# Masthetheus/kmer-ml

Measured on NVIDIA B200. Metric: kmer_count_feature_throughput, higher is better.
Workload: dtype u32

## Files before the change

### kmerml_b200/csrc/api.cu

```cuda
#include <dlfcn.h>

#include <algorithm>
#include <atomic>
#include <condition_variable>
#include <cstdio>
#include <cstdlib>
#include <cstring>
#include <memory>
#include <mutex>
#include <new>
#include <string>
#include <thread>
#include <vector>

#include "internal.h"

namespace km {

static thread_local std::string g_err;
void set_error(const std::string& msg) { g_err = msg; }
int cuda_fail(cudaError_t e, const char* what) {
    g_err = std::string("CUDA error: ") + cudaGetErrorString(e) + " in " + what;
    return KMERML_ERR_CUDA;
}
// ... 229 lines not shown
    lm.scratch_stride = scratch_stride;
    if (scratch_stride) {
        rc = ws.scratch.ensure((size_t)scratch_stride * lm.scratch_slots * 4);
        if (rc) return rc;
    }
    lm.scratch = (uint32_t*)ws.scratch.p;

    const uint64_t total_bytes = h_offsets[n_genomes] - h_offsets[0];
    const uint64_t target = (uint64_t)ctx->sm_count * 8;
    uint64_t walked_bytes = total_bytes;
    if (range_end) walked_bytes = std::min(total_bytes, range_end > range_begin ? range_end - range_begin : 0);
    int part_tiles_per_slice = 1;
    {
        const uint64_t tiles = std::max<uint64_t>(walked_bytes / TILE_BYTES, 1);
        const uint64_t slots = (uint64_t)ctx->sm_count * 2;
        for (uint64_t w = 1;; w++) {
            const uint64_t t = (tiles * 100 + slots * w * 96 - 1) / (slots * w * 96);
            if (t <= (uint64_t)PART_MAX_TILES_PER_RUN) {
                part_tiles_per_slice = (int)std::max<uint64_t>(t, 1);
                break;
            }
        }
    }
    if (const char* e = getenv("KMERML_TILES_PER_RUN")) {
        const int v = atoi(e);
        if (v >= 1 && v <= PART_MAX_TILES_PER_RUN) part_tiles_per_slice = v;
    }
    std::vector<uint64_t> slice_bytes(n_genomes);
    std::vector<uint32_t> first_slice(n_genomes + 1);
    uint64_t n_slices = 0;
    for (int g = 0; g < n_genomes; g++) {
        uint64_t bytes = h_offsets[g + 1] - h_offsets[g];
        uint64_t sb;
        if (use_part) {
            sb = (uint64_t)TILE_BYTES * part_tiles_per_slice;
// ... 93 lines not shown
    const size_t row_bytes = (size_t)row.off[nk] * 4;
    if (use_part) {
        const int k_stop = std::max(kcount - PART_LOW_BASES, kmin);
        uint64_t max_group_runs = 0, max_group_bytes = 0, max_group_genomes = 0;
        for (size_t gi = 0, g0 = 0; gi < group_end.size(); g0 = group_end[gi], gi++) {
            max_group_runs = std::max<uint64_t>(max_group_runs, first_slice[group_end[gi]] - first_slice[g0]);
            max_group_bytes = std::max<uint64_t>(max_group_bytes, h_offsets[group_end[gi]] - h_offsets[g0]);
            max_group_genomes = std::max<uint64_t>(max_group_genomes, group_end[gi] - g0);
        }
        const int nb = 1 << (2 * (kcount - PART_LOW_BASES));
        const size_t payload_bytes = align_up((size_t)max_group_runs * run_payload_bytes, 256);
        const size_t nsec_bytes = align_up((size_t)max_group_runs * nb * 2, 256);
        const size_t ov_bytes = align_up((size_t)max_group_bytes * 4 + 64, 256);
        const size_t ovc_bytes = align_up((size_t)n_genomes * 8 + 8, 256);
        const size_t tl_bytes = align_up((size_t)((max_group_bytes >> 6) + 1024 * (max_group_genomes + 1)) * 8, 256);
        rc = ws.part.ensure(payload_bytes + nsec_bytes + ov_bytes + tl_bytes + ovc_bytes);
        if (rc) return rc;
        uint8_t* pw = (uint8_t*)ws.part.p;
        void* d_payload = pw;
        uint16_t* d_nsec = (uint16_t*)(pw + payload_bytes);
        uint32_t* d_overflow = (uint32_t*)(pw + payload_bytes + nsec_bytes);
        unsigned long long* d_tail_list = (unsigned long long*)(pw + payload_bytes + nsec_bytes + ov_bytes);
        unsigned int* d_ov_counts = (unsigned int*)(pw + payload_bytes + nsec_bytes + ov_bytes + tl_bytes);
        unsigned int* d_tail_counts = d_ov_counts + n_genomes;
        unsigned int* d_tail_any = d_tail_counts + n_genomes;
        KM_CUDA(cudaMemsetAsync(d_ov_counts, 0, (size_t)n_genomes * 8 + 8, s));
        for (int i = 0; i < nk; i++)
            if (row.k[i] < k_stop)
                KM_CUDA(cudaMemset2DAsync(d_counts + row.off[i], (size_t)counts_stride * 4, 0,
                                          (size_t)(1ull << (2 * row.k[i])) * 4, (size_t)n_genomes, s));
        if (scratch_stride && k_stop > kmin)
            KM_CUDA(cudaMemsetAsync(lm.scratch, 0, (size_t)scratch_stride * n_genomes * 4, s));
        int g0 = 0;
        for (size_t gi = 0; gi < group_end.size(); gi++) {
            const int g1 = group_end[gi], ng = g1 - g0;
            const int nt = (int)(first_slice[g1] - first_slice[g0]);
            const uint64_t batch_lo = h_offsets[g0];
            {
                Prof pr(ctx, s, 4, nt > 0 ? 1 : 0);
                rc = launch_partition(d_fasta, d_genomes, d_slices + first_slice[g0], nt, part_tiles_per_slice, kcount,
                                      kmin, min_rec, lm, d_stats, d_payload, d_nsec, d_overflow, d_ov_counts, batch_lo,
                                      d_tail_list, d_tail_counts, d_tail_any, (uint32_t)g0, s);
            }
            if (rc) return rc;
            {
                Prof pr(ctx, s, 5, 1);
                rc = launch_bucket(lm, row, kcount, kmin, d_gruns, part_tiles_per_slice, d_payload, d_nsec, d_stats,
                                   canonical ? nullptr : d_freq, freq_stride, d_totals, (uint32_t)g0, ng, s);
            }
            if (rc) return rc;
            if (kcount > kmin) {
                Prof pr(ctx, s, 3, canonical || !d_freq ? 2 : 4);
                rc = launch_tails(d_fasta, lm, row, kcount, kmin, min_rec, d_genomes, d_slices + first_slice[g0], nt,
                                  d_tail_list, d_tail_counts, d_tail_any, batch_lo, d_stats, canonical ? nullptr : d_freq, freq_stride,
                                  (uint32_t)g0, ng, s);
                if (rc) return rc;
            }
            for (int h0 = g0; h0 < g1; h0 += 32768) {
                const int nh = std::min(32768, g1 - h0);
                {
                    Prof pr(ctx, s, 3, canonical || !d_freq ? 1 : 2);
                    rc = launch_overflow(lm, row, kcount, kmin, d_genomes, d_overflow, d_ov_counts, batch_lo, d_stats,
                                         canonical ? nullptr : d_freq, freq_stride, (uint32_t)h0, nh, s);
// ... 1292 lines not shown
```

### kmerml_b200/csrc/dense.cu

```cuda
#include <algorithm>

#include "fasta_walk.cuh"
#include "internal.h"

namespace km {

struct DevTails {
    const LevelMap* lm;
    GenomeStats* st;
    uint32_t genome;
    __device__ __noinline__ void tail(int j, uint32_t idx) const {
        atomicAdd(lm->ptr(genome, j) + idx, 1u);
        atomicAdd(&st->n_tail[j], 1ull);
    }
};

struct NoTails {
    __device__ __forceinline__ void tail(int, uint32_t) const {}
};

struct TailList {
    unsigned long long* list;
    unsigned int* counts;
    unsigned int* any_full;
    uint64_t batch_lo;
    uint32_t genome0;
};
__device__ __forceinline__ unsigned long long* tail_list_of(const TailList& tl, const GenomeDev& gd, uint32_t g,
                                                            uint32_t* cap) {
    *cap = (uint32_t)((gd.hi - gd.file_lo) >> 6) + 1024u;
    return tl.list + ((gd.file_lo - tl.batch_lo) >> 6) + 1024ull * (g - tl.genome0);
}
struct ListTails {
    const LevelMap* lm;
    GenomeStats* st;
    uint32_t genome;
    int k_stop;
    unsigned long long* list;
    unsigned int* count;
    unsigned int* any_full;
    uint32_t cap;
    __device__ __noinline__ void tail(int j, uint32_t idx) const {
        atomicAdd(&st->n_tail[j], 1ull);
        if (j < k_stop) {
            atomicAdd(lm->ptr(genome, j) + idx, 1u);
            return;
        }
// ... 555 lines not shown
struct PartWalkSmem {
    uint32_t last16[COUNT_THREADS];
    uint8_t flags[2 * COUNT_THREADS];
    uint8_t clean[COUNT_THREADS];
};

template <int NB_SHIFT>
struct PartSmem {
    uint16_t staged[PartGeom<NB_SHIFT>::stage_entries];
    uint32_t cnt[PART_MAX_BUCKETS];
    uint16_t written[PART_MAX_BUCKETS];
    PartWalkSmem walk;
    unsigned long long carry[2];
    uint32_t prev_tile[2];
    unsigned long long sh_total;
};
static_assert(sizeof(PartSmem<10>) <= 113 * 1024, "two partition CTAs must fit in one SM's shared memory");

struct GenomeRuns {
    uint32_t run0, n_runs;
};

__device__ __forceinline__ void store_sector(uint4* dst, const uint4& a, const uint4& b) {
    asm volatile("st.global.v8.b32 [%0], {%1, %2, %3, %4, %5, %6, %7, %8};" ::"l"(dst), "r"(a.x), "r"(a.y), "r"(a.z),
                 "r"(a.w), "r"(b.x), "r"(b.y), "r"(b.z), "r"(b.w) : "memory");
}

template <int NB_SHIFT>
__device__ __noinline__ void flush_slot_slow(PartSmem<NB_SHIFT>& sm, uint32_t b, uint4* region, uint32_t cap,
                                             uint32_t* ov, unsigned int* ov_count) {
// ... 9 lines not shown
            region[((size_t)b * cap + wr) * 2 + 1] = slot[2 * q + 1];
            wr++;
        } else {
            overflow_push_sector(ov, ov_count, b, slot16 + q * PART_SECTOR);
        }
    }
    if (nfull && left) {
        const uint4 a = slot[2 * nfull], d = slot[2 * nfull + 1];
        slot[0] = a;
        slot[1] = d;
    }
    sm.written[b] = (uint16_t)wr;
    sm.cnt[b] = left;
}

template <int NB_SHIFT>
__global__ void __launch_bounds__(COUNT_THREADS, 2)
partition_kernel(const uint8_t* __restrict__ buf, const GenomeDev* __restrict__ gds,
                 const Slice* __restrict__ runs, DenseParams P, LevelMap lm,
                 GenomeStats* stats, uint4* __restrict__ payload, uint16_t* __restrict__ nsec, uint32_t cap,
                 uint32_t* __restrict__ overflow, unsigned int* __restrict__ ov_counts, uint64_t batch_lo,
                 TailList tl, int k_stop) {
    using G = PartGeom<NB_SHIFT>;
    constexpr uint32_t slot_size = G::slot_size;
    constexpr uint32_t nb = G::nb;
    constexpr uint32_t VPB = slot_size / 8;
    extern __shared__ __align__(16) unsigned char part_smem_raw[];
    PartSmem<NB_SHIFT>& sm = *reinterpret_cast<PartSmem<NB_SHIFT>*>(part_smem_raw);
    const int tid = threadIdx.x;
    const Slice sl = runs[blockIdx.x];
    const GenomeDev gd = gds[sl.genome];
    Genome g;
    g.b = buf;
    g.lo = gd.lo;
    g.hi = gd.hi;
    TileCtx tc;
    tc.flags = sm.walk.flags; tc.clean = sm.walk.clean; tc.last16 = sm.walk.last16;
    tc.carry = sm.carry; tc.prev_tile = sm.prev_tile;
    for (uint32_t i = tid; i < nb; i += COUNT_THREADS) { sm.cnt[i] = 0; sm.written[i] = 0; }
    if (tid == 0) sm.sh_total = 0;

    SlotSink<NB_SHIFT> sink;
    sink.cnt_s = (uint32_t)__cvta_generic_to_shared(sm.cnt);
    sink.staged_s = (uint32_t)__cvta_generic_to_shared(sm.staged);
    sink.ov = overflow + (gd.file_lo - batch_lo);
    sink.ov_count = ov_counts + sl.genome;
    sink.kmask = P.mask;
    sink.n = 0;
    ListTails tails;
    tails.lm = &lm; tails.st = stats + sl.genome; tails.genome = sl.genome; tails.k_stop = k_stop;
    tails.list = tail_list_of(tl, gd, sl.genome, &tails.cap);
    tails.count = tl.counts + sl.genome;
    tails.any_full = tl.any_full;
    uint4* const region = payload + (size_t)blockIdx.x * nb * cap * 2;
    walk_slice<false>(buf, g, sl, P, sink, tails, tc, [&](uint32_t) {
        uint4* st = reinterpret_cast<uint4*>(sm.staged);
        if (G::owned) {
#pragma unroll
            for (int h = 0; h < 2; h++) {
                const uint32_t b = (uint32_t)tid + h * COUNT_THREADS;
                const uint32_t c = sm.cnt[b];
                if (c < PART_SECTOR) continue;
                const uint32_t wr = sm.written[b];
                if (c > slot_size || wr + 3u > cap) {
                    flush_slot_slow<NB_SHIFT>(sm, b, region, cap, sink.ov, sink.ov_count);
                    continue;
                }
                const uint32_t sw = ((uint32_t)tid >> 2) & 1u, sx = sw ^ 1u;
                uint4* slot = st + b * VPB;
                uint4* dst = region + (b * cap + wr) * 2u;
                {
                    const uint4 x0 = slot[sw], x1 = slot[sx];
                    dst[sw] = x0;
                    dst[sx] = x1;
                }
                uint32_t mv = 2;
                if (c >= 2 * PART_SECTOR) {
                    const uint4 x0 = slot[2 + sw], x1 = slot[2 + sx];
                    dst[2 + sw] = x0;
                    dst[2 + sx] = x1;
                    mv = 4;
                    if (c == 3 * PART_SECTOR) {
                        const uint4 y0 = slot[4 + sw], y1 = slot[4 + sx];
                        dst[4 + sw] = y0;
                        dst[4 + sx] = y1;
                        mv = 0;
                    }
                }
                const uint4 m0 = slot[mv + sw], m1 = slot[mv + sx];
                slot[sw] = m0;
                slot[sx] = m1;
                sm.written[b] = (uint16_t)(wr + c / PART_SECTOR);
                sm.cnt[b] = c % PART_SECTOR;
            }
        } else {
#pragma unroll
            for (int j = 0; j < (int)(G::stage_entries / 8 / COUNT_THREADS); j++) {
                const uint32_t v = (uint32_t)tid + j * COUNT_THREADS;
                const uint32_t b = v / VPB, jv = v % VPB, q = jv >> 1;
                const uint32_t c = min(sm.cnt[b], slot_size);
                const uint32_t nfull = c / PART_SECTOR;
                const uint32_t wr = sm.written[b];
                const uint4 x = st[v];
                if (VPB <= 32) __syncwarp(); else __syncthreads();
                if (q < nfull) {
                    const uint32_t sec = wr + q;
                    if (sec < cap) region[(b * cap + sec) * 2u + (jv & 1u)] = x;
                    else if (!(jv & 1u)) overflow_push_sector(sink.ov, sink.ov_count, b, sm.staged + b * slot_size + q * PART_SECTOR);
                }
                if (VPB <= 32) __syncwarp(); else __syncthreads();
                if (q == nfull && nfull && (c % PART_SECTOR)) st[b * VPB + (jv & 1u)] = x;
                if (jv == 0) {
                    sm.cnt[b] = c % PART_SECTOR;
                    sm.written[b] = (uint16_t)min(wr + nfull, cap);
                }
            }
        }
    });
    __syncthreads();
    for (uint32_t b = tid; b < nb; b += COUNT_THREADS) {
        const uint32_t left = sm.cnt[b];
        uint32_t wr = sm.written[b];
        if (left) {
            uint32_t e[PART_SECTOR / 2];
            const uint16_t* src16 = sm.staged + (size_t)b * slot_size;
            const uint32_t* src = reinterpret_cast<const uint32_t*>(src16);
            if (wr < cap) {
#pragma unroll
                for (int i = 0; i < PART_SECTOR / 2; i++) {
                    uint32_t w = src[i];
                    const uint32_t pad = payload_pad(b, b * 16u + 2u * i);
                    if (2u * i >= left) w = (w & 0xFFFF0000u) | pad;
                    if (2u * i + 1u >= left) w = (w & 0x0000FFFFu) | ((pad ^ 1u) << 16);
                    e[i] = w;
                }
                uint4* dst = region + (b * cap + wr) * 2u;
                dst[0] = make_uint4(e[0], e[1], e[2], e[3]);
                dst[1] = make_uint4(e[4], e[5], e[6], e[7]);
                wr++;
            } else {
                for (uint32_t i = 0; i < left; i++)
                    overflow_push(sink.ov, sink.ov_count, (b << (2 * PART_LOW)) | (src16[i] & (uint32_t)(PART_BINS - 1)));
            }
        }
        nsec[(size_t)blockIdx.x * nb + b] = (uint16_t)wr;
    }
    const unsigned long long total = block_sum_u32(sink.n, &sm.sh_total);
    if (tid == 0 && total) atomicAdd(&stats[sl.genome].total_top, total);
}

struct LevelInfo {
    int ki[16];
};

constexpr int BUCKET_THREADS = 512;

constexpr int BUCKET_NS_CHUNK = 1024;
#ifndef KM_BUCKET_BULK_STORE
#define KM_BUCKET_BULK_STORE 1
#endif
struct BucketSmem {
    uint32_t hist[PART_BINS + 256];
    uint16_t ns[BUCKET_NS_CHUNK];
    unsigned long long tot[16];
    uint32_t* lvl_counts[16];
    float* lvl_freq[16];
    double lvl_inv[16];
};
constexpr int BUCKET_CTAS_PER_SM = 3;
static_assert(sizeof(BucketSmem) <= 75 * 1024, "three bucket CTAs must fit in one SM's shared memory");

__device__ __forceinline__ void bulk_store(void* dst, uint32_t src_smem, uint32_t bytes) {
    asm volatile("cp.async.bulk.global.shared::cta.bulk_group [%0], [%1], %2;" ::"l"(dst), "r"(src_smem), "r"(bytes) : "memory");
    asm volatile("cp.async.bulk.commit_group;" ::: "memory");
}
__device__ __forceinline__ void bulk_store_wait_read() { asm volatile("cp.async.bulk.wait_group.read 0;" ::: "memory"); }

__device__ __forceinline__ void hist_add8(uint32_t hbase, const uint4& x, uint32_t fix) {
    const uint32_t w[4] = {x.x ^ fix, x.y ^ fix, x.z ^ fix, x.w ^ fix};
#pragma unroll
    for (int i = 0; i < 4; i++) {
        asm volatile("red.shared.add.u32 [%0], 1;" ::"r"(hbase + ((w[i] & 0xFFFFu) << 2)) : "memory");
        asm volatile("red.shared.add.u32 [%0], 1;" ::"r"(hbase + ((w[i] >> 16) << 2)) : "memory");
    }
}

__global__ void __launch_bounds__(BUCKET_THREADS, BUCKET_CTAS_PER_SM)
bucket_kernel(LevelMap lm, RowSpec row, LevelInfo li, int k, int k_stop, const GenomeRuns* __restrict__ grs,
              const uint4* __restrict__ payload, const uint16_t* __restrict__ nsec, uint32_t cap,
              const GenomeStats* __restrict__ stats, float* freq, uint64_t freq_stride, uint64_t* totals,
              uint32_t genome0) {
    extern __shared__ __align__(16) unsigned char bucket_smem_raw[];
    BucketSmem& sm = *reinterpret_cast<BucketSmem*>(bucket_smem_raw);
    const int tid = threadIdx.x;
    const uint32_t b = blockIdx.x;
    const uint32_t nb = gridDim.x;
    const uint32_t g = genome0 + blockIdx.y;
    const GenomeRuns gr = grs[g];
    if (tid < row.nk) {
        const int j = row.k[tid];
        unsigned long long t = stats[g].total_top;
        for (int i = j; i < k; i++) t += stats[g].n_tail[i];
        sm.tot[tid] = t;
        if (totals && b == 0) totals[(uint64_t)g * row.nk + tid] = t;
    }
    __syncthreads();
    if (tid >= 32 && tid < 48) {
        const int level = tid - 32;
        uint32_t* cp = nullptr;
        float* fp = nullptr;
        double inv = 0.0;
        if (level >= k_stop && level <= k) {
// ... 12 lines not shown
    constexpr int PER1 = PART_BINS / 4 / BUCKET_THREADS;
    constexpr int PER2 = PART_BINS / 16 / BUCKET_THREADS;
    const uint32_t hbase = (uint32_t)__cvta_generic_to_shared(sm.hist);
    const uint32_t fix = payload_fix(b);
    {
        uint4* h4 = reinterpret_cast<uint4*>(sm.hist);
        for (int i = tid; i < (PART_BINS + 256) / 4; i += BUCKET_THREADS) h4[i] = make_uint4(0, 0, 0, 0);
    }
    constexpr int NWARP = BUCKET_THREADS / 32;
    const int lane = tid & 31, wid = tid >> 5;
    const size_t run_stride = (size_t)nb * cap * 2;
    for (uint32_t rb = 0; rb < gr.n_runs; rb += BUCKET_NS_CHUNK) {
        const uint32_t nr = min(gr.n_runs - rb, (uint32_t)BUCKET_NS_CHUNK);
        __syncthreads();
        for (uint32_t i = tid; i < nr; i += BUCKET_THREADS)
            sm.ns[i] = __ldg(nsec + (size_t)(gr.run0 + rb + i) * nb + b);
        __syncthreads();
        const uint4* base = payload + ((size_t)(gr.run0 + rb) * nb + b) * cap * 2;
        uint32_t r = wid, c = 0, nv = 0;
        auto settle = [&]() {
            while (r < nr && 32u * c >= (nv = 2u * sm.ns[r])) { r += NWARP; c = 0; }
        };
        auto issue = [&](uint4& x, bool& live) -> bool {
            settle();
            if (r >= nr) { live = false; return false; }
            const uint32_t v = 32u * c + lane;
            live = v < nv;
            if (live) x = __ldg(base + (size_t)r * run_stride + v);
            c++;
            return true;
        };
        uint4 x0, x1, x2, x3;
        bool l0, l1, l2, l3;
// ... 80 lines not shown
        float* fl = sm.lvl_freq[level];
        const double invl = sm.lvl_inv[level];
        for (int i = tid; i < n_next; i += 32) {
            const uint4 c = reinterpret_cast<const uint4*>(cur)[i];
            const uint32_t v = c.x + c.y + c.z + c.w;
            cl[i] = v;
            if (fl) fl[i] = (float)((double)v * invl);
            nxt[i] = v;
        }
        __syncwarp();
        uint32_t* t = cur; cur = nxt; nxt = t;
        n_cur = n_next;
    }
}

constexpr int OV_TABLE = 4096;
constexpr uint32_t OV_EMPTY = 0xFFFFFFFFu;

__global__ void __launch_bounds__(256)
overflow_kernel(LevelMap lm, RowSpec row, LevelInfo li, int k, int k_stop, const GenomeDev* __restrict__ gds,
                const uint32_t* __restrict__ overflow, const unsigned int* __restrict__ ov_counts, uint64_t batch_lo,
                const GenomeStats* __restrict__ stats, float* freq, uint64_t freq_stride, uint32_t genome0, int pass) {
    __shared__ uint32_t t_key[OV_TABLE];
    __shared__ uint32_t t_cnt[OV_TABLE];
    __shared__ unsigned int t_used;
    const uint32_t g = genome0 + blockIdx.y;
    const unsigned int n = ov_counts[g];
    if (blockIdx.x * 256u >= n) return;
    const uint32_t* ov = overflow + (gds[g].file_lo - batch_lo);
    const int tid = threadIdx.x;
// ... 315 lines not shown
                const uint32_t own = tile[t][A][B];
                out[b] = x < rc ? own + tile[p][Br][Ar] : (x == rc ? own : 0u);
            }
            *reinterpret_cast<uint4*>(c + x0) = make_uint4(out[0], out[1], out[2], out[3]);
            if (f)
                *reinterpret_cast<float4*>(f + x0) = make_float4((float)((double)out[0] * inv), (float)((double)out[1] * inv),
                                                                 (float)((double)out[2] * inv), (float)((double)out[3] * inv));
        }
    }
}

int dense_setup_attributes() {
    KM_CUDA(cudaFuncSetAttribute(count_kernel<1>, cudaFuncAttributeMaxDynamicSharedMemorySize,
                                 (1 << (2 * SMEM_MAX_K)) * 4));
    KM_CUDA(cudaFuncSetAttribute(count8_kernel, cudaFuncAttributeMaxDynamicSharedMemorySize, 32768 * 4));
    KM_CUDA(cudaFuncSetAttribute(partition_kernel<10>, cudaFuncAttributeMaxDynamicSharedMemorySize, (int)sizeof(PartSmem<10>)));
    KM_CUDA(cudaFuncSetAttribute(partition_kernel<8>, cudaFuncAttributeMaxDynamicSharedMemorySize, (int)sizeof(PartSmem<8>)));
    KM_CUDA(cudaFuncSetAttribute(partition_kernel<6>, cudaFuncAttributeMaxDynamicSharedMemorySize, (int)sizeof(PartSmem<6>)));
    KM_CUDA(cudaFuncSetAttribute(partition_kernel<4>, cudaFuncAttributeMaxDynamicSharedMemorySize, (int)sizeof(PartSmem<4>)));
    KM_CUDA(cudaFuncSetAttribute(bucket_kernel, cudaFuncAttributeMaxDynamicSharedMemorySize, (int)sizeof(BucketSmem)));
    return KMERML_OK;
}

int launch_prologue(const uint8_t* d_fasta, const uint64_t* d_offsets, GenomeDev* d_genomes,
                    GenomeStats* d_stats, int n_genomes, cudaStream_t s) {
    if (n_genomes <= 0) return KMERML_OK;
    prologue_kernel<<<(n_genomes + 127) / 128, 128, 0, s>>>(d_fasta, d_offsets, d_genomes, d_stats, n_genomes);
    KM_CUDA(cudaGetLastError());
    return KMERML_OK;
}

static DenseParams make_params(int k, int min_rec, bool tails, int tail_lo) {
    DenseParams P;
    P.k = k;
    P.mask = k >= 16 ? 0xFFFFFFFFu : ((1u << (2 * k)) - 1u);
// ... 27 lines not shown
        count_kernel<0><<<n_slices, COUNT_THREADS, 0, s>>>(d_fasta, d_genomes, d_slices, P, lm, d_stats, nullptr);
    }
    KM_CUDA(cudaGetLastError());
    return KMERML_OK;
}

uint32_t part_region_cap(int k, int tiles_per_run) {
    const uint32_t nb = 1u << (2 * (k - PART_LOW));
    return (uint32_t)tiles_per_run * (2u * TILE_BYTES / PART_SECTOR) / nb;
}

int launch_partition(const uint8_t* d_fasta, const GenomeDev* d_genomes, const Slice* d_runs, int n_runs,
                     int tiles_per_run, int k, int k_bottom, int min_rec, const LevelMap& lm,
                     GenomeStats* d_stats, void* d_payload, uint16_t* d_nsec, uint32_t* d_overflow,
                     unsigned int* d_ov_counts, uint64_t batch_lo, unsigned long long* d_tail_list,
                     unsigned int* d_tail_counts, unsigned int* d_tail_any, uint32_t genome0, cudaStream_t s) {
    if (n_runs <= 0) return KMERML_OK;
    DenseParams P = make_params(k, min_rec, k > k_bottom, k_bottom);
    const int k_stop = std::max(k - PART_LOW, k_bottom);
    const uint32_t cap = part_region_cap(k, tiles_per_run);
    TailList tl;
    tl.list = d_tail_list; tl.counts = d_tail_counts; tl.batch_lo = batch_lo; tl.genome0 = genome0;
    tl.any_full = d_tail_any;
#define KM_LAUNCH_PART(NBS)                                                                           \
    partition_kernel<NBS><<<n_runs, COUNT_THREADS, sizeof(PartSmem<NBS>), s>>>(                       \
        d_fasta, d_genomes, d_runs, P, lm, d_stats, (uint4*)d_payload, d_nsec, cap, d_overflow,       \
        d_ov_counts, batch_lo, tl, k_stop)
    switch (2 * (k - PART_LOW)) {
        case 10: KM_LAUNCH_PART(10); break;
        case 8: KM_LAUNCH_PART(8); break;
        case 6: KM_LAUNCH_PART(6); break;
        default: KM_LAUNCH_PART(4); break;
    }
#undef KM_LAUNCH_PART
    KM_CUDA(cudaGetLastError());
    return KMERML_OK;
}

static LevelInfo make_level_info(const RowSpec& row) {
    LevelInfo li;
    for (int j = 0; j < 16; j++) {
        li.ki[j] = -1;
        for (int i = 0; i < row.nk; i++)
            if (row.k[i] == j) li.ki[j] = i;
    }
    return li;
}

int launch_bucket(const LevelMap& lm, const RowSpec& row, int k, int k_bottom, const void* d_genome_runs,
                  int tiles_per_run, const void* d_payload, const uint16_t* d_nsec, const GenomeStats* d_stats,
                  float* d_freq, uint64_t freq_stride, uint64_t* d_totals, uint32_t genome0, int n_genomes,
                  cudaStream_t s) {
    if (n_genomes <= 0) return KMERML_OK;
    const int nb = 1 << (2 * (k - PART_LOW));
    const LevelInfo li = make_level_info(row);
    const int k_stop = std::max(k - PART_LOW, k_bottom);
    const uint32_t cap = part_region_cap(k, tiles_per_run);
    for (int h0 = 0; h0 < n_genomes; h0 += 32768) {
        dim3 grid((unsigned)nb, (unsigned)std::min(32768, n_genomes - h0));
        bucket_kernel<<<grid, BUCKET_THREADS, sizeof(BucketSmem), s>>>(lm, row, li, k, k_stop,
            (const GenomeRuns*)d_genome_runs, (const uint4*)d_payload, d_nsec, cap, d_stats, d_freq, freq_stride,
            d_totals, genome0 + (uint32_t)h0);
        KM_CUDA(cudaGetLastError());
    }
    return KMERML_OK;
}

int launch_overflow(const LevelMap& lm, const RowSpec& row, int k, int k_bottom, const GenomeDev* d_genomes,
                    const uint32_t* d_overflow, const unsigned int* d_ov_counts, uint64_t batch_lo,
                    const GenomeStats* d_stats, float* d_freq, uint64_t freq_stride, uint32_t genome0, int n_genomes,
                    cudaStream_t s) {
    if (n_genomes <= 0) return KMERML_OK;
    const LevelInfo li = make_level_info(row);
    const int k_stop = std::max(k - PART_LOW, k_bottom);
    dim3 grid(64, (unsigned)n_genomes);
    for (int pass = 0; pass < (d_freq ? 2 : 1); pass++) {
        overflow_kernel<<<grid, 256, 0, s>>>(lm, row, li, k, k_stop, d_genomes, d_overflow, d_ov_counts, batch_lo,
// ... 114 lines not shown
```

### kmerml_b200/csrc/internal.h

```cpp
#pragma once
#include <cuda_runtime.h>
#include <stdint.h>

#include <algorithm>
#include <functional>
#include <string>

#include "../../include/kmerml_b200.h"

namespace km {

void set_error(const std::string& msg);
int cuda_fail(cudaError_t e, const char* what);
#define KM_CUDA(expr)                                        \
    do {                                                     \
        cudaError_t e__ = (expr);                            \
        if (e__ != cudaSuccess) return ::km::cuda_fail(e__, #expr); \
    } while (0)

struct GenomeDev {
    uint64_t file_lo;
    uint64_t lo;
    uint64_t hi;
};
// ... 45 lines not shown
int launch_slice_headers(const uint8_t* d_fasta, const GenomeDev* d_genomes, Slice* d_slices, int n_slices,
                         cudaStream_t s);
int launch_count(const uint8_t* d_fasta, const GenomeDev* d_genomes, const Slice* d_slices,
                 int n_slices, int k, int k_bottom, int min_rec, bool use_smem, const LevelMap& lm,
                 GenomeStats* d_stats, cudaStream_t s);
int launch_cascade(const LevelMap& lm, int k_top, int k_bottom, uint32_t genome0, int n_genomes,
                   cudaStream_t s);
int cascade_launches(int k_top, int k_bottom);
int finalize_launches(const RowSpec& row, bool canonical);
int launch_finalize(const LevelMap& lm, const RowSpec& row, int k_top, bool canonical,
                    const GenomeStats* d_stats, float* d_freq, uint64_t freq_stride,
                    uint64_t* d_totals, uint32_t genome0, int n_genomes, cudaStream_t s);
constexpr int PART_MIN_K = 9, PART_MAX_K = 12, PART_LOW_BASES = 7;
constexpr int PART_STAGE_ENTRIES = 32768;
constexpr int PART_MAX_TILES_PER_RUN = 64;
uint32_t part_region_cap(int k, int tiles_per_run);
int launch_partition(const uint8_t* d_fasta, const GenomeDev* d_genomes, const Slice* d_runs, int n_runs,
                     int tiles_per_run, int k, int k_bottom, int min_rec, const LevelMap& lm,
                     GenomeStats* d_stats, void* d_payload, uint16_t* d_nsec, uint32_t* d_overflow,
                     unsigned int* d_ov_counts, uint64_t batch_lo, unsigned long long* d_tail_list,
                     unsigned int* d_tail_counts, unsigned int* d_tail_any, uint32_t genome0, cudaStream_t s);
int launch_tails(const uint8_t* d_fasta, const LevelMap& lm, const RowSpec& row, int k, int k_bottom, int min_rec,
                 const GenomeDev* d_genomes, const Slice* d_tiles, int n_tiles, unsigned long long* d_tail_list,
                 unsigned int* d_tail_counts, unsigned int* d_tail_any, uint64_t batch_lo, const GenomeStats* d_stats,
                 float* d_freq, uint64_t freq_stride, uint32_t genome0, int n_genomes, cudaStream_t s);
int launch_bucket(const LevelMap& lm, const RowSpec& row, int k, int k_bottom, const void* d_genome_runs,
                  int tiles_per_run, const void* d_payload, const uint16_t* d_nsec, const GenomeStats* d_stats,
                  float* d_freq, uint64_t freq_stride, uint64_t* d_totals, uint32_t genome0, int n_genomes,
                  cudaStream_t s);
int launch_overflow(const LevelMap& lm, const RowSpec& row, int k, int k_bottom, const GenomeDev* d_genomes,
                    const uint32_t* d_overflow, const unsigned int* d_ov_counts, uint64_t batch_lo,
                    const GenomeStats* d_stats, float* d_freq, uint64_t freq_stride, uint32_t genome0, int n_genomes,
                    cudaStream_t s);
int launch_finalize_low(const LevelMap& lm, const RowSpec& row, int k_top, int level_limit,
                        const GenomeStats* d_stats, float* d_freq, uint64_t freq_stride, uint32_t genome0,
                        int n_genomes, cudaStream_t s);
int launch_encode(const uint8_t* d_fasta, const GenomeDev* d_genomes, const Slice* d_slices, int n_slices,
                  uint8_t* d_symbols, cudaStream_t s);
int launch_first_occurrence(const uint8_t* d_fasta, const GenomeDev* d_genomes, const Slice* d_slices,
                            int n_slices, int k, int min_rec, uint32_t* d_first, cudaStream_t s);
int dense_setup_attributes();

struct NarrowSpec {
    int n, n_small;
// ... 121 lines not shown
```

Before: 251.1.

## Add SM-gated persistent work claiming for partition and bucket kernels

```diff
diff --git a/kmerml_b200/csrc/api.cu b/kmerml_b200/csrc/api.cu
--- a/kmerml_b200/csrc/api.cu
+++ b/kmerml_b200/csrc/api.cu
@@ -267,11 +267,15 @@
     {
         const uint64_t tiles = std::max<uint64_t>(walked_bytes / TILE_BYTES, 1);
         const uint64_t slots = (uint64_t)ctx->sm_count * 2;
-        for (uint64_t w = 1;; w++) {
-            const uint64_t t = (tiles * 100 + slots * w * 96 - 1) / (slots * w * 96);
-            if (t <= (uint64_t)PART_MAX_TILES_PER_RUN) {
-                part_tiles_per_slice = (int)std::max<uint64_t>(t, 1);
-                break;
+        if (tiles >= slots * 16 * PART_LONG_BATCH_TILES_PER_RUN) {
+            part_tiles_per_slice = PART_LONG_BATCH_TILES_PER_RUN;
+        } else {
+            for (uint64_t w = 1;; w++) {
+                const uint64_t t = (tiles * 100 + slots * w * 96 - 1) / (slots * w * 96);
+                if (t <= (uint64_t)PART_MAX_TILES_PER_RUN) {
+                    part_tiles_per_slice = (int)std::max<uint64_t>(t, 1);
+                    break;
+                }
             }
         }
     }
@@ -395,7 +399,8 @@
         const size_t ov_bytes = align_up((size_t)max_group_bytes * 4 + 64, 256);
         const size_t ovc_bytes = align_up((size_t)n_genomes * 8 + 8, 256);
         const size_t tl_bytes = align_up((size_t)((max_group_bytes >> 6) + 1024 * (max_group_genomes + 1)) * 8, 256);
-        rc = ws.part.ensure(payload_bytes + nsec_bytes + ov_bytes + tl_bytes + ovc_bytes);
+        const size_t claim_bytes = 256;
+        rc = ws.part.ensure(payload_bytes + nsec_bytes + ov_bytes + tl_bytes + ovc_bytes + claim_bytes);
         if (rc) return rc;
         uint8_t* pw = (uint8_t*)ws.part.p;
         void* d_payload = pw;
@@ -405,6 +410,17 @@
         unsigned int* d_ov_counts = (unsigned int*)(pw + payload_bytes + nsec_bytes + ov_bytes + tl_bytes);
         unsigned int* d_tail_counts = d_ov_counts + n_genomes;
         unsigned int* d_tail_any = d_tail_counts + n_genomes;
+        unsigned int* d_claim = (unsigned int*)(pw + payload_bytes + nsec_bytes + ov_bytes + tl_bytes + ovc_bytes);
+        SmGate part_gate{d_claim, 0, ~0u, ctx->sm_count}, bucket_gate{d_claim + 2, 0, ~0u, ctx->sm_count};
+        bool gated = false;
+        if (const char* e = getenv("KMERML_PART_SMS")) {
+            const int v = atoi(e);
+            if (v >= 0 && v <= ctx->sm_count) {
+                part_gate.sm_hi = (uint32_t)v;
+                bucket_gate.sm_lo = (uint32_t)v;
+                gated = true;
+            }
+        }
         KM_CUDA(cudaMemsetAsync(d_ov_counts, 0, (size_t)n_genomes * 8 + 8, s));
         for (int i = 0; i < nk; i++)
             if (row.k[i] < k_stop)
@@ -421,13 +437,13 @@
                 Prof pr(ctx, s, 4, nt > 0 ? 1 : 0);
                 rc = launch_partition(d_fasta, d_genomes, d_slices + first_slice[g0], nt, part_tiles_per_slice, kcount,
                                       kmin, min_rec, lm, d_stats, d_payload, d_nsec, d_overflow, d_ov_counts, batch_lo,
-                                      d_tail_list, d_tail_counts, d_tail_any, (uint32_t)g0, s);
+                                      d_tail_list, d_tail_counts, d_tail_any, (uint32_t)g0, gated ? &part_gate : nullptr, s);
             }
             if (rc) return rc;
             {
                 Prof pr(ctx, s, 5, 1);
                 rc = launch_bucket(lm, row, kcount, kmin, d_gruns, part_tiles_per_slice, d_payload, d_nsec, d_stats,
-                                   canonical ? nullptr : d_freq, freq_stride, d_totals, (uint32_t)g0, ng, s);
+                                   canonical ? nullptr : d_freq, freq_stride, d_totals, (uint32_t)g0, ng, gated ? &bucket_gate : nullptr, s);
             }
             if (rc) return rc;
             if (kcount > kmin) {
diff --git a/kmerml_b200/csrc/dense.cu b/kmerml_b200/csrc/dense.cu
--- a/kmerml_b200/csrc/dense.cu
+++ b/kmerml_b200/csrc/dense.cu
@@ -31,6 +31,22 @@
     *cap = (uint32_t)((gd.hi - gd.file_lo) >> 6) + 1024u;
     return tl.list + ((gd.file_lo - tl.batch_lo) >> 6) + 1024ull * (g - tl.genome0);
 }
+struct WorkClaim {
+    unsigned int* next;
+    uint32_t sm_lo, sm_hi;
+};
+__device__ __forceinline__ bool claim_sm_allowed(const WorkClaim& w) {
+    uint32_t id;
+    asm volatile("mov.u32 %0, %%smid;" : "=r"(id));
+    const bool ok = id >= w.sm_lo && id < w.sm_hi;
+    if (ok) atomicExch(w.next + 1, 1u);
+    return ok;
+}
+__device__ __forceinline__ uint32_t claim_item(const WorkClaim& w, bool allowed) {
+    if (!allowed && *(volatile unsigned int*)(w.next + 1)) return ~0u;
+    return atomicAdd(w.next, 1u);
+}
+
 struct ListTails {
     const LevelMap* lm;
     GenomeStats* st;
@@ -616,6 +632,7 @@
     unsigned long long carry[2];
     uint32_t prev_tile[2];
     unsigned long long sh_total;
+    uint32_t run;
 };
 static_assert(sizeof(PartSmem<10>) <= 113 * 1024, "two partition CTAs must fit in one SM's shared memory");
 
@@ -655,13 +672,13 @@
     sm.cnt[b] = left;
 }
 
-template <int NB_SHIFT>
+template <int NB_SHIFT, bool CLAIM>
 __global__ void __launch_bounds__(COUNT_THREADS, 2)
 partition_kernel(const uint8_t* __restrict__ buf, const GenomeDev* __restrict__ gds,
                  const Slice* __restrict__ runs, DenseParams P, LevelMap lm,
                  GenomeStats* stats, uint4* __restrict__ payload, uint16_t* __restrict__ nsec, uint32_t cap,
                  uint32_t* __restrict__ overflow, unsigned int* __restrict__ ov_counts, uint64_t batch_lo,
-                 TailList tl, int k_stop) {
+                 TailList tl, int k_stop, WorkClaim wc, uint32_t n_runs) {
     using G = PartGeom<NB_SHIFT>;
     constexpr uint32_t slot_size = G::slot_size;
     constexpr uint32_t nb = G::nb;
@@ -669,125 +686,140 @@
     extern __shared__ __align__(16) unsigned char part_smem_raw[];
     PartSmem<NB_SHIFT>& sm = *reinterpret_cast<PartSmem<NB_SHIFT>*>(part_smem_raw);
     const int tid = threadIdx.x;
-    const Slice sl = runs[blockIdx.x];
-    const GenomeDev gd = gds[sl.genome];
-    Genome g;
-    g.b = buf;
-    g.lo = gd.lo;
-    g.hi = gd.hi;
-    TileCtx tc;
-    tc.flags = sm.walk.flags; tc.clean = sm.walk.clean; tc.last16 = sm.walk.last16;
-    tc.carry = sm.carry; tc.prev_tile = sm.prev_tile;
-    for (uint32_t i = tid; i < nb; i += COUNT_THREADS) { sm.cnt[i] = 0; sm.written[i] = 0; }
-    if (tid == 0) sm.sh_total = 0;
-
-    SlotSink<NB_SHIFT> sink;
-    sink.cnt_s = (uint32_t)__cvta_generic_to_shared(sm.cnt);
-    sink.staged_s = (uint32_t)__cvta_generic_to_shared(sm.staged);
-    sink.ov = overflow + (gd.file_lo - batch_lo);
-    sink.ov_count = ov_counts + sl.genome;
-    sink.kmask = P.mask;
-    sink.n = 0;
-    ListTails tails;
-    tails.lm = &lm; tails.st = stats + sl.genome; tails.genome = sl.genome; tails.k_stop = k_stop;
-    tails.list = tail_list_of(tl, gd, sl.genome, &tails.cap);
-    tails.count = tl.counts + sl.genome;
-    tails.any_full = tl.any_full;
-    uint4* const region = payload + (size_t)blockIdx.x * nb * cap * 2;
-    walk_slice<false>(buf, g, sl, P, sink, tails, tc, [&](uint32_t) {
-        uint4* st = reinterpret_cast<uint4*>(sm.staged);
-        if (G::owned) {
-#pragma unroll
-            for (int h = 0; h < 2; h++) {
-                const uint32_t b = (uint32_t)tid + h * COUNT_THREADS;
-                const uint32_t c = sm.cnt[b];
-                if (c < PART_SECTOR) continue;
-                const uint32_t wr = sm.written[b];
-                if (c > slot_size || wr + 3u > cap) {
-                    flush_slot_slow<NB_SHIFT>(sm, b, region, cap, sink.ov, sink.ov_count);
-                    continue;
+    bool allowed = false;
+    if constexpr (CLAIM) allowed = tid == 0 && claim_sm_allowed(wc);
+    for (;;) {
+        if constexpr (CLAIM) {
+            __syncthreads();
+            if (tid == 0) sm.run = claim_item(wc, allowed);
+            __syncthreads();
+            if (sm.run >= n_runs) break;
+        }
+        auto run_no = [&]() -> uint32_t { return CLAIM ? sm.run : blockIdx.x; };
+        const Slice sl = runs[run_no()];
+        const GenomeDev gd = gds[sl.genome];
+        Genome g;
+        g.b = buf;
+        g.lo = gd.lo;
+        g.hi = gd.hi;
+        TileCtx tc;
+        tc.flags = sm.walk.flags; tc.clean = sm.walk.clean; tc.last16 = sm.walk.last16;
+        tc.carry = sm.carry; tc.prev_tile = sm.prev_tile;
+        for (uint32_t i = tid; i < nb; i += COUNT_THREADS) { sm.cnt[i] = 0; sm.written[i] = 0; }
+        if (tid == 0) sm.sh_total = 0;
+
+        SlotSink<NB_SHIFT> sink;
+        sink.cnt_s = (uint32_t)__cvta_generic_to_shared(sm.cnt);
+        sink.staged_s = (uint32_t)__cvta_generic_to_shared(sm.staged);
+        sink.ov = overflow + (gd.file_lo - batch_lo);
+        sink.ov_count = ov_counts + sl.genome;
+        sink.kmask = P.mask;
+        sink.n = 0;
+        ListTails tails;
+        tails.lm = &lm; tails.st = stats + sl.genome; tails.genome = sl.genome; tails.k_stop = k_stop;
+        tails.list = tail_list_of(tl, gd, sl.genome, &tails.cap);
+        tails.count = tl.counts + sl.genome;
+        tails.any_full = tl.any_full;
+        uint4* const region0 = CLAIM ? nullptr : payload + (size_t)blockIdx.x * nb * cap * 2;
+        auto run_region = [&]() { return CLAIM ? payload + (size_t)sm.run * nb * cap * 2 : region0; };
+        walk_slice<false>(buf, g, sl, P, sink, tails, tc, [&](uint32_t) {
+            uint4* const region = run_region();
+            uint4* st = reinterpret_cast<uint4*>(sm.staged);
+            if (G::owned) {
+#pragma unroll
+                for (int h = 0; h < 2; h++) {
+                    const uint32_t b = (uint32_t)tid + h * COUNT_THREADS;
+                    const uint32_t c = sm.cnt[b];
+                    if (c < PART_SECTOR) continue;
+                    const uint32_t wr = sm.written[b];
+                    if (c > slot_size || wr + 3u > cap) {
+                        flush_slot_slow<NB_SHIFT>(sm, b, region, cap, sink.ov, sink.ov_count);
+                        continue;
+                    }
+                    const uint32_t sw = ((uint32_t)tid >> 2) & 1u, sx = sw ^ 1u;
+                    uint4* slot = st + b * VPB;
+                    uint4* dst = region + (b * cap + wr) * 2u;
+                    {
+                        const uint4 x0 = slot[sw], x1 = slot[sx];
+                        dst[sw] = x0;
+                        dst[sx] = x1;
+                    }
+                    uint32_t mv = 2;
+                    if (c >= 2 * PART_SECTOR) {
+                        const uint4 x0 = slot[2 + sw], x1 = slot[2 + sx];
+                        dst[2 + sw] = x0;
+                        dst[2 + sx] = x1;
+                        mv = 4;
+                        if (c == 3 * PART_SECTOR) {
+                            const uint4 y0 = slot[4 + sw], y1 = slot[4 + sx];
+                            dst[4 + sw] = y0;
+                            dst[4 + sx] = y1;
+                            mv = 0;
+                        }
+                    }
+                    const uint4 m0 = slot[mv + sw], m1 = slot[mv + sx];
+                    slot[sw] = m0;
+                    slot[sx] = m1;
+                    sm.written[b] = (uint16_t)(wr + c / PART_SECTOR);
+                    sm.cnt[b] = c % PART_SECTOR;
                 }
-                const uint32_t sw = ((uint32_t)tid >> 2) & 1u, sx = sw ^ 1u;
-                uint4* slot = st + b * VPB;
-                uint4* dst = region + (b * cap + wr) * 2u;
-                {
-                    const uint4 x0 = slot[sw], x1 = slot[sx];
-                    dst[sw] = x0;
-                    dst[sx] = x1;
-                }
-                uint32_t mv = 2;
-                if (c >= 2 * PART_SECTOR) {
-                    const uint4 x0 = slot[2 + sw], x1 = slot[2 + sx];
-                    dst[2 + sw] = x0;
-                    dst[2 + sx] = x1;
-                    mv = 4;
-                    if (c == 3 * PART_SECTOR) {
-                        const uint4 y0 = slot[4 + sw], y1 = slot[4 + sx];
-                        dst[4 + sw] = y0;
-                        dst[4 + sx] = y1;
-                        mv = 0;
+            } else {
+#pragma unroll
+                for (int j = 0; j < (int)(G::stage_entries / 8 / COUNT_THREADS); j++) {
+                    const uint32_t v = (uint32_t)tid + j * COUNT_THREADS;
+                    const uint32_t b = v / VPB, jv = v % VPB, q = jv >> 1;
+                    const uint32_t c = min(sm.cnt[b], slot_size);
+                    const uint32_t nfull = c / PART_SECTOR;
+                    const uint32_t wr = sm.written[b];
+                    const uint4 x = st[v];
+                    if (VPB <= 32) __syncwarp(); else __syncthreads();
+                    if (q < nfull) {
+                        const uint32_t sec = wr + q;
+                        if (sec < cap) region[(b * cap + sec) * 2u + (jv & 1u)] = x;
+                        else if (!(jv & 1u)) overflow_push_sector(sink.ov, sink.ov_count, b, sm.staged + b * slot_size + q * PART_SECTOR);
+                    }
+                    if (VPB <= 32) __syncwarp(); else __syncthreads();
+                    if (q == nfull && nfull && (c % PART_SECTOR)) st[b * VPB + (jv & 1u)] = x;
+                    if (jv == 0) {
+                        sm.cnt[b] = c % PART_SECTOR;
+                        sm.written[b] = (uint16_t)min(wr + nfull, cap);
                     }
                 }
-                const uint4 m0 = slot[mv + sw], m1 = slot[mv + sx];
-                slot[sw] = m0;
-                slot[sx] = m1;
-                sm.written[b] = (uint16_t)(wr + c / PART_SECTOR);
-                sm.cnt[b] = c % PART_SECTOR;
             }
-        } else {
-#pragma unroll
-            for (int j = 0; j < (int)(G::stage_entries / 8 / COUNT_THREADS); j++) {
-                const uint32_t v = (uint32_t)tid + j * COUNT_THREADS;
-                const uint32_t b = v / VPB, jv = v % VPB, q = jv >> 1;
-                const uint32_t c = min(sm.cnt[b], slot_size);
-                const uint32_t nfull = c / PART_SECTOR;
-                const uint32_t wr = sm.written[b];
-                const uint4 x = st[v];
-                if (VPB <= 32) __syncwarp(); else __syncthreads();
-                if (q < nfull) {
-                    const uint32_t sec = wr + q;
-                    if (sec < cap) region[(b * cap + sec) * 2u + (jv & 1u)] = x;
-                    else if (!(jv & 1u)) overflow_push_sector(sink.ov, sink.ov_count, b, sm.staged + b * slot_size + q * PART_SECTOR);
-                }
-                if (VPB <= 32) __syncwarp(); else __syncthreads();
-                if (q == nfull && nfull && (c % PART_SECTOR)) st[b * VPB + (jv & 1u)] = x;
-                if (jv == 0) {
-                    sm.cnt[b] = c % PART_SECTOR;
-                    sm.written[b] = (uint16_t)min(wr + nfull, cap);
+        });
+        __syncthreads();
+        uint4* const region = run_region();
+        for (uint32_t b = tid; b < nb; b += COUNT_THREADS) {
+            const uint32_t left = sm.cnt[b];
+            uint32_t wr = sm.written[b];
+            if (left) {
+                uint32_t e[PART_SECTOR / 2];
+                const uint16_t* src16 = sm.staged + (size_t)b * slot_size;
+                const uint32_t* src = reinterpret_cast<const uint32_t*>(src16);
+                if (wr < cap) {
+#pragma unroll
+                    for (int i = 0; i < PART_SECTOR / 2; i++) {
+                        uint32_t w = src[i];
+                        const uint32_t pad = payload_pad(b, b * 16u + 2u * i);
+                        if (2u * i >= left) w = (w & 0xFFFF0000u) | pad;
+                        if (2u * i + 1u >= left) w = (w & 0x0000FFFFu) | ((pad ^ 1u) << 16);
+                        e[i] = w;
+                    }
+                    uint4* dst = region + (b * cap + wr) * 2u;
+                    dst[0] = make_uint4(e[0], e[1], e[2], e[3]);
+                    dst[1] = make_uint4(e[4], e[5], e[6], e[7]);
+                    wr++;
+                } else {
+                    for (uint32_t i = 0; i < left; i++)
+                        overflow_push(sink.ov, sink.ov_count, (b << (2 * PART_LOW)) | (src16[i] & (uint32_t)(PART_BINS - 1)));
                 }
             }
-        }
-    });
-    __syncthreads();
-    for (uint32_t b = tid; b < nb; b += COUNT_THREADS) {
-        const uint32_t left = sm.cnt[b];
-        uint32_t wr = sm.written[b];
-        if (left) {
-            uint32_t e[PART_SECTOR / 2];
-            const uint16_t* src16 = sm.staged + (size_t)b * slot_size;
-            const uint32_t* src = reinterpret_cast<const uint32_t*>(src16);
-            if (wr < cap) {
-#pragma unroll
-                for (int i = 0; i < PART_SECTOR / 2; i++) {
-                    uint32_t w = src[i];
-                    const uint32_t pad = payload_pad(b, b * 16u + 2u * i);
-                    if (2u * i >= left) w = (w & 0xFFFF0000u) | pad;
-                    if (2u * i + 1u >= left) w = (w & 0x0000FFFFu) | ((pad ^ 1u) << 16);
-                    e[i] = w;
-                }
-                uint4* dst = region + (b * cap + wr) * 2u;
-                dst[0] = make_uint4(e[0], e[1], e[2], e[3]);
-                dst[1] = make_uint4(e[4], e[5], e[6], e[7]);
-                wr++;
-            } else {
-                for (uint32_t i = 0; i < left; i++)
-                    overflow_push(sink.ov, sink.ov_count, (b << (2 * PART_LOW)) | (src16[i] & (uint32_t)(PART_BINS - 1)));
-            }
-        }
-        nsec[(size_t)blockIdx.x * nb + b] = (uint16_t)wr;
-    }
-    const unsigned long long total = block_sum_u32(sink.n, &sm.sh_total);
-    if (tid == 0 && total) atomicAdd(&stats[sl.genome].total_top, total);
+            nsec[(size_t)run_no() * nb + b] = (uint16_t)wr;
+        }
+        const unsigned long long total = block_sum_u32(sink.n, &sm.sh_total);
+        if (tid == 0 && total) atomicAdd(&stats[sl.genome].total_top, total);
+        if constexpr (!CLAIM) break;
+    }
 }
 
 struct LevelInfo {
@@ -807,6 +839,7 @@
     uint32_t* lvl_counts[16];
     float* lvl_freq[16];
     double lvl_inv[16];
+    uint32_t item, next_item;
 };
 constexpr int BUCKET_CTAS_PER_SM = 3;
 static_assert(sizeof(BucketSmem) <= 75 * 1024, "three bucket CTAs must fit in one SM's shared memory");
@@ -826,17 +859,16 @@
     }
 }
 
-__global__ void __launch_bounds__(BUCKET_THREADS, BUCKET_CTAS_PER_SM)
-bucket_kernel(LevelMap lm, RowSpec row, LevelInfo li, int k, int k_stop, const GenomeRuns* __restrict__ grs,
-              const uint4* __restrict__ payload, const uint16_t* __restrict__ nsec, uint32_t cap,
-              const GenomeStats* __restrict__ stats, float* freq, uint64_t freq_stride, uint64_t* totals,
-              uint32_t genome0) {
-    extern __shared__ __align__(16) unsigned char bucket_smem_raw[];
-    BucketSmem& sm = *reinterpret_cast<BucketSmem*>(bucket_smem_raw);
+template <bool CLAIM>
+__device__ __forceinline__ void bucket_item(BucketSmem& sm, const LevelMap& lm, const RowSpec& row, const LevelInfo& li,
+                                            int k, int k_stop, const GenomeRuns* __restrict__ grs,
+                                            const uint4* __restrict__ payload, const uint16_t* __restrict__ nsec,
+                                            uint32_t cap, const GenomeStats* __restrict__ stats, float* freq,
+                                            uint64_t freq_stride, uint64_t* totals, uint32_t genome0) {
     const int tid = threadIdx.x;
-    const uint32_t b = blockIdx.x;
-    const uint32_t nb = gridDim.x;
-    const uint32_t g = genome0 + blockIdx.y;
+    const uint32_t nb_shift = 2u * (uint32_t)(k - PART_LOW), nb = 1u << nb_shift;
+    auto item_b = [&]() -> uint32_t { return CLAIM ? sm.item & (nb - 1u) : blockIdx.x; };
+    const uint32_t b = item_b(), g = genome0 + (CLAIM ? sm.item >> nb_shift : blockIdx.y);
     const GenomeRuns gr = grs[g];
     if (tid < row.nk) {
         const int j = row.k[tid];
@@ -879,9 +911,9 @@
         const uint32_t nr = min(gr.n_runs - rb, (uint32_t)BUCKET_NS_CHUNK);
         __syncthreads();
         for (uint32_t i = tid; i < nr; i += BUCKET_THREADS)
-            sm.ns[i] = __ldg(nsec + (size_t)(gr.run0 + rb + i) * nb + b);
+            sm.ns[i] = __ldg(nsec + (size_t)(gr.run0 + rb + i) * nb + item_b());
         __syncthreads();
-        const uint4* base = payload + ((size_t)(gr.run0 + rb) * nb + b) * cap * 2;
+        const uint4* base = payload + ((size_t)(gr.run0 + rb) * nb + item_b()) * cap * 2;
         uint32_t r = wid, c = 0, nv = 0;
         auto settle = [&]() {
             while (r < nr && 32u * c >= (nv = 2u * sm.ns[r])) { r += NWARP; c = 0; }
@@ -992,6 +1024,31 @@
     }
 }
 
+template <bool CLAIM>
+__global__ void __launch_bounds__(BUCKET_THREADS, BUCKET_CTAS_PER_SM)
+bucket_kernel(LevelMap lm, RowSpec row, LevelInfo li, int k, int k_stop, const GenomeRuns* __restrict__ grs,
+              const uint4* __restrict__ payload, const uint16_t* __restrict__ nsec, uint32_t cap,
+              const GenomeStats* __restrict__ stats, float* freq, uint64_t freq_stride, uint64_t* totals,
+              uint32_t genome0, uint32_t n_items, WorkClaim wc) {
+    extern __shared__ __align__(16) unsigned char bucket_smem_raw[];
+    BucketSmem& sm = *reinterpret_cast<BucketSmem*>(bucket_smem_raw);
+    if constexpr (!CLAIM) {
+        bucket_item<false>(sm, lm, row, li, k, k_stop, grs, payload, nsec, cap, stats, freq, freq_stride, totals, genome0);
+        return;
+    }
+    const int tid = threadIdx.x;
+    const bool allowed = tid == 0 && claim_sm_allowed(wc);
+    if (tid == 0) sm.item = claim_item(wc, allowed);
+    __syncthreads();
+    while (sm.item < n_items) {
+        if (tid == 0) sm.next_item = claim_item(wc, allowed);
+        bucket_item<true>(sm, lm, row, li, k, k_stop, grs, payload, nsec, cap, stats, freq, freq_stride, totals, genome0);
+        __syncthreads();
+        if (tid == 0) sm.item = sm.next_item;
+        __syncthreads();
+    }
+}
+
 constexpr int OV_TABLE = 4096;
 constexpr uint32_t OV_EMPTY = 0xFFFFFFFFu;
 
@@ -1337,11 +1394,16 @@
     KM_CUDA(cudaFuncSetAttribute(count_kernel<1>, cudaFuncAttributeMaxDynamicSharedMemorySize,
                                  (1 << (2 * SMEM_MAX_K)) * 4));
     KM_CUDA(cudaFuncSetAttribute(count8_kernel, cudaFuncAttributeMaxDynamicSharedMemorySize, 32768 * 4));
-    KM_CUDA(cudaFuncSetAttribute(partition_kernel<10>, cudaFuncAttributeMaxDynamicSharedMemorySize, (int)sizeof(PartSmem<10>)));
-    KM_CUDA(cudaFuncSetAttribute(partition_kernel<8>, cudaFuncAttributeMaxDynamicSharedMemorySize, (int)sizeof(PartSmem<8>)));
-    KM_CUDA(cudaFuncSetAttribute(partition_kernel<6>, cudaFuncAttributeMaxDynamicSharedMemorySize, (int)sizeof(PartSmem<6>)));
-    KM_CUDA(cudaFuncSetAttribute(partition_kernel<4>, cudaFuncAttributeMaxDynamicSharedMemorySize, (int)sizeof(PartSmem<4>)));
-    KM_CUDA(cudaFuncSetAttribute(bucket_kernel, cudaFuncAttributeMaxDynamicSharedMemorySize, (int)sizeof(BucketSmem)));
+    KM_CUDA(cudaFuncSetAttribute(partition_kernel<10, false>, cudaFuncAttributeMaxDynamicSharedMemorySize, (int)sizeof(PartSmem<10>)));
+    KM_CUDA(cudaFuncSetAttribute(partition_kernel<10, true>, cudaFuncAttributeMaxDynamicSharedMemorySize, (int)sizeof(PartSmem<10>)));
+    KM_CUDA(cudaFuncSetAttribute(partition_kernel<8, false>, cudaFuncAttributeMaxDynamicSharedMemorySize, (int)sizeof(PartSmem<8>)));
+    KM_CUDA(cudaFuncSetAttribute(partition_kernel<8, true>, cudaFuncAttributeMaxDynamicSharedMemorySize, (int)sizeof(PartSmem<8>)));
+    KM_CUDA(cudaFuncSetAttribute(partition_kernel<6, false>, cudaFuncAttributeMaxDynamicSharedMemorySize, (int)sizeof(PartSmem<6>)));
+    KM_CUDA(cudaFuncSetAttribute(partition_kernel<6, true>, cudaFuncAttributeMaxDynamicSharedMemorySize, (int)sizeof(PartSmem<6>)));
+    KM_CUDA(cudaFuncSetAttribute(partition_kernel<4, false>, cudaFuncAttributeMaxDynamicSharedMemorySize, (int)sizeof(PartSmem<4>)));
+    KM_CUDA(cudaFuncSetAttribute(partition_kernel<4, true>, cudaFuncAttributeMaxDynamicSharedMemorySize, (int)sizeof(PartSmem<4>)));
+    KM_CUDA(cudaFuncSetAttribute(bucket_kernel<false>, cudaFuncAttributeMaxDynamicSharedMemorySize, (int)sizeof(BucketSmem)));
+    KM_CUDA(cudaFuncSetAttribute(bucket_kernel<true>, cudaFuncAttributeMaxDynamicSharedMemorySize, (int)sizeof(BucketSmem)));
     return KMERML_OK;
 }
 
@@ -1399,7 +1461,8 @@
                      int tiles_per_run, int k, int k_bottom, int min_rec, const LevelMap& lm,
                      GenomeStats* d_stats, void* d_payload, uint16_t* d_nsec, uint32_t* d_overflow,
                      unsigned int* d_ov_counts, uint64_t batch_lo, unsigned long long* d_tail_list,
-                     unsigned int* d_tail_counts, unsigned int* d_tail_any, uint32_t genome0, cudaStream_t s) {
+                     unsigned int* d_tail_counts, unsigned int* d_tail_any, uint32_t genome0, const SmGate* gate,
+                     cudaStream_t s) {
     if (n_runs <= 0) return KMERML_OK;
     DenseParams P = make_params(k, min_rec, k > k_bottom, k_bottom);
     const int k_stop = std::max(k - PART_LOW, k_bottom);
@@ -1407,10 +1470,16 @@
     TailList tl;
     tl.list = d_tail_list; tl.counts = d_tail_counts; tl.batch_lo = batch_lo; tl.genome0 = genome0;
     tl.any_full = d_tail_any;
-#define KM_LAUNCH_PART(NBS)                                                                           \
-    partition_kernel<NBS><<<n_runs, COUNT_THREADS, sizeof(PartSmem<NBS>), s>>>(                       \
-        d_fasta, d_genomes, d_runs, P, lm, d_stats, (uint4*)d_payload, d_nsec, cap, d_overflow,       \
-        d_ov_counts, batch_lo, tl, k_stop)
+    WorkClaim wc{nullptr, 0, 0};
+    if (gate) {
+        wc = WorkClaim{gate->claim, gate->sm_lo, gate->sm_hi};
+        KM_CUDA(cudaMemsetAsync(gate->claim, 0, 2 * sizeof(unsigned int), s));
+    }
+    const int grid = gate ? std::min(n_runs, 2 * gate->n_sms) : n_runs;
+#define KM_LAUNCH_PART(NBS)                                                                                        \
+    (gate ? partition_kernel<NBS, true> : partition_kernel<NBS, false>)<<<grid, COUNT_THREADS, sizeof(PartSmem<NBS>), s>>>( \
+        d_fasta, d_genomes, d_runs, P, lm, d_stats, (uint4*)d_payload, d_nsec, cap, d_overflow,                    \
+        d_ov_counts, batch_lo, tl, k_stop, wc, (uint32_t)n_runs)
     switch (2 * (k - PART_LOW)) {
         case 10: KM_LAUNCH_PART(10); break;
         case 8: KM_LAUNCH_PART(8); break;
@@ -1435,17 +1504,31 @@
 int launch_bucket(const LevelMap& lm, const RowSpec& row, int k, int k_bottom, const void* d_genome_runs,
                   int tiles_per_run, const void* d_payload, const uint16_t* d_nsec, const GenomeStats* d_stats,
                   float* d_freq, uint64_t freq_stride, uint64_t* d_totals, uint32_t genome0, int n_genomes,
-                  cudaStream_t s) {
+                  const SmGate* gate, cudaStream_t s) {
     if (n_genomes <= 0) return KMERML_OK;
     const int nb = 1 << (2 * (k - PART_LOW));
     const LevelInfo li = make_level_info(row);
     const int k_stop = std::max(k - PART_LOW, k_bottom);
     const uint32_t cap = part_region_cap(k, tiles_per_run);
+    if (gate) {
+        if ((uint64_t)nb * (uint64_t)n_genomes >= (1ull << 32)) {
+            set_error("too many genomes in one group of the partition path");
+            return KMERML_ERR_RANGE;
+        }
+        const uint32_t n_items = (uint32_t)nb * (uint32_t)n_genomes;
+        KM_CUDA(cudaMemsetAsync(gate->claim, 0, 2 * sizeof(unsigned int), s));
+        const unsigned grid = std::min<uint32_t>(n_items, (uint32_t)(BUCKET_CTAS_PER_SM * gate->n_sms));
+        bucket_kernel<true><<<grid, BUCKET_THREADS, sizeof(BucketSmem), s>>>(lm, row, li, k, k_stop,
+            (const GenomeRuns*)d_genome_runs, (const uint4*)d_payload, d_nsec, cap, d_stats, d_freq, freq_stride,
+            d_totals, genome0, n_items, WorkClaim{gate->claim, gate->sm_lo, gate->sm_hi});
+        KM_CUDA(cudaGetLastError());
+        return KMERML_OK;
+    }
     for (int h0 = 0; h0 < n_genomes; h0 += 32768) {
         dim3 grid((unsigned)nb, (unsigned)std::min(32768, n_genomes - h0));
-        bucket_kernel<<<grid, BUCKET_THREADS, sizeof(BucketSmem), s>>>(lm, row, li, k, k_stop,
+        bucket_kernel<false><<<grid, BUCKET_THREADS, sizeof(BucketSmem), s>>>(lm, row, li, k, k_stop,
             (const GenomeRuns*)d_genome_runs, (const uint4*)d_payload, d_nsec, cap, d_stats, d_freq, freq_stride,
-            d_totals, genome0 + (uint32_t)h0);
+            d_totals, genome0 + (uint32_t)h0, 0u, WorkClaim{nullptr, 0, 0});
         KM_CUDA(cudaGetLastError());
     }
     return KMERML_OK;
diff --git a/kmerml_b200/csrc/internal.h b/kmerml_b200/csrc/internal.h
--- a/kmerml_b200/csrc/internal.h
+++ b/kmerml_b200/csrc/internal.h
@@ -83,12 +83,19 @@
 constexpr int PART_MIN_K = 9, PART_MAX_K = 12, PART_LOW_BASES = 7;
 constexpr int PART_STAGE_ENTRIES = 32768;
 constexpr int PART_MAX_TILES_PER_RUN = 64;
+constexpr int PART_LONG_BATCH_TILES_PER_RUN = 32;
 uint32_t part_region_cap(int k, int tiles_per_run);
+struct SmGate {
+    unsigned int* claim;
+    uint32_t sm_lo, sm_hi;
+    int n_sms;
+};
 int launch_partition(const uint8_t* d_fasta, const GenomeDev* d_genomes, const Slice* d_runs, int n_runs,
                      int tiles_per_run, int k, int k_bottom, int min_rec, const LevelMap& lm,
                      GenomeStats* d_stats, void* d_payload, uint16_t* d_nsec, uint32_t* d_overflow,
                      unsigned int* d_ov_counts, uint64_t batch_lo, unsigned long long* d_tail_list,
-                     unsigned int* d_tail_counts, unsigned int* d_tail_any, uint32_t genome0, cudaStream_t s);
+                     unsigned int* d_tail_counts, unsigned int* d_tail_any, uint32_t genome0, const SmGate* gate,
+                     cudaStream_t s);
 int launch_tails(const uint8_t* d_fasta, const LevelMap& lm, const RowSpec& row, int k, int k_bottom, int min_rec,
                  const GenomeDev* d_genomes, const Slice* d_tiles, int n_tiles, unsigned long long* d_tail_list,
                  unsigned int* d_tail_counts, unsigned int* d_tail_any, uint64_t batch_lo, const GenomeStats* d_stats,
@@ -96,7 +103,7 @@
 int launch_bucket(const LevelMap& lm, const RowSpec& row, int k, int k_bottom, const void* d_genome_runs,
                   int tiles_per_run, const void* d_payload, const uint16_t* d_nsec, const GenomeStats* d_stats,
                   float* d_freq, uint64_t freq_stride, uint64_t* d_totals, uint32_t genome0, int n_genomes,
-                  cudaStream_t s);
+                  const SmGate* gate, cudaStream_t s);
 int launch_overflow(const LevelMap& lm, const RowSpec& row, int k, int k_bottom, const GenomeDev* d_genomes,
                     const uint32_t* d_overflow, const unsigned int* d_ov_counts, uint64_t batch_lo,
                     const GenomeStats* d_stats, float* d_freq, uint64_t freq_stride, uint32_t genome0, int n_genomes,
```

After: 254.6 (median of 6 runs). 1.01x the previous value.
